# greysun/GraphEmbeddings

Measured on AMD Instinct MI355X. Metric: scored triples/sec/GPU (d=200), higher is better.
Workload: dtype f32

## Files before the change

### graphembeddings_amd/csrc/ge_common.h

```cpp
#pragma once
#include <hip/hip_runtime.h>
#include <hip/hip_ext.h>
#include <stdint.h>

#include <initializer_list>

#include "../../include/ge_hip.h"

namespace ge {

constexpr int kWave = 64;
constexpr int kBlock = 256;
constexpr int kMaxBlocks = 256 * 8;

template <int VEC> struct Vec;
template <> struct Vec<1> { using type = float; };
template <> struct Vec<2> { using type = float2; };
template <> struct Vec<4> { using type = float4; };

template <int VEC>
__device__ __forceinline__ void load_vec(const float* __restrict__ p, float (&r)[VEC]) {
  if constexpr (VEC == 4) {
    float4 v = *reinterpret_cast<const float4*>(p);
    r[0] = v.x; r[1] = v.y; r[2] = v.z; r[3] = v.w;
  } else if constexpr (VEC == 2) {
    float2 v = *reinterpret_cast<const float2*>(p);
    r[0] = v.x; r[1] = v.y;
  } else {
    r[0] = *p;
  }
}

template <int VEC>
__device__ __forceinline__ void store_vec(float* __restrict__ p, const float (&r)[VEC]) {
  if constexpr (VEC == 4) {
    *reinterpret_cast<float4*>(p) = make_float4(r[0], r[1], r[2], r[3]);
  } else if constexpr (VEC == 2) {
    *reinterpret_cast<float2*>(p) = make_float2(r[0], r[1]);
  } else {
    *p = r[0];
  }
}

template <int LPT>
__device__ __forceinline__ float group_sum(float v) {
#pragma unroll
  for (int m = LPT / 2; m >= 1; m >>= 1) v += __shfl_xor(v, m, kWave);
  return v;
}

__device__ __forceinline__ float clip_scale(float ss, float max_norm, float& inv) {
  inv = rsqrtf(ss);
  return fminf(inv, 1.0f / max_norm) * max_norm;
}

__device__ __forceinline__ float sigmoidf_dev(float x) { return 1.0f / (1.0f + expf(-x)); }

__device__ __forceinline__ void atomic_add_f32(float* p, float v) {
  __hip_atomic_fetch_add(p, v, __ATOMIC_RELAXED, __HIP_MEMORY_SCOPE_AGENT);
}

inline int grid_for(int64_t units, int units_per_block) {
  int64_t g = (units + units_per_block - 1) / units_per_block;
  if (g < 1) g = 1;
  if (g > kMaxBlocks) g = kMaxBlocks;
  return (int)g;
}

inline int launch_status() {
  hipError_t e = hipGetLastError();
  return e == hipSuccess ? 0 : (int)e;
}

inline size_t align_up(size_t v, size_t a) { return (v + a - 1) / a * a; }

inline unsigned sort_key_bits(int64_t n) {
  unsigned b = 1;
  while (b < 32 && ((uint64_t)1 << b) <= (uint64_t)n) ++b;
  return b;
}

inline bool aligned16(std::initializer_list<const void*> ptrs) {
  for (const void* p : ptrs) if ((uintptr_t)p & 15) return false;
  return true;
}

__device__ __forceinline__ uint32_t philox_w0(uint32_t c0, uint32_t c1, uint32_t c2, uint32_t c3,
                                              uint32_t k0, uint32_t k1) {
#pragma unroll
  for (int r = 0; r < 10; ++r) {
    uint64_t p0 = (uint64_t)0xD2511F53u * c0, p1 = (uint64_t)0xCD9E8D57u * c2;
    uint32_t n0 = (uint32_t)(p1 >> 32) ^ c1 ^ k0, n1 = (uint32_t)p1;
    uint32_t n2 = (uint32_t)(p0 >> 32) ^ c3 ^ k1, n3 = (uint32_t)p0;
    c0 = n0; c1 = n1; c2 = n2; c3 = n3;
// ... 50 lines not shown
```

### graphembeddings_amd/csrc/ge_complex.hip

```cpp
#include "ge_complex_dev.h"
#include "ge_launch.h"

namespace ge {

template <bool SPEC, int VEC, int LPT, int NITER>
__global__ __launch_bounds__(kBlock) void complex_score_kernel(
    const float* __restrict__ table, int64_t N, int d, const int32_t* __restrict__ triples, int64_t B,
    float max_norm, int apply_sigmoid, float* __restrict__ out, float label, float l2,
    const float* __restrict__ table_sumsq, int64_t ld) {
  constexpr int GPW = kWave / LPT;
  const int lane = threadIdx.x & (kWave - 1), sub = lane % LPT, grp = lane / LPT;
  const int64_t wave = ((int64_t)blockIdx.x * blockDim.x + threadIdx.x) >> 6;
  const int64_t nwaves = ((int64_t)gridDim.x * blockDim.x) >> 6;
  const int k = d >> 1, nvec = k / VEC;
  const float wscale = 1.0f / (float)d;
  for (int64_t base = wave * GPW; base < B; base += nwaves * GPW) {
    const int64_t g = base + grp;
    const bool live = g < B;
    int32_t hi = 0, ti = 0, ri = 0;
    if (live) { hi = triples[3 * g]; ti = triples[3 * g + 1]; ri = triples[3 * g + 2]; }
    const bool bad = bad3(N, hi, ti, ri);
    if (bad) { hi = ti = ri = 0; }
    Row<VEC, NITER> h, t, r;
    load_row_at<VEC, LPT, NITER>(table + (int64_t)hi * ld, k, nvec, sub, h);
// ... 118 lines not shown
          graw<SPEC, VEC, NITER>(X, xn[0], xn[1], xn[2], it, v, sub == 0, gre, gim);
          nre_[v] = kn.alpha * gre + kn.beta * xn[X].re[it][v];
          nim_[v] = kn.alpha * gim + kn.beta * xn[X].im[it][v];
        }
        if (same) {
#pragma unroll
          for (int v = 0; v < VEC; ++v) { pre_[v] += nre_[v]; pim_[v] += nim_[v]; }
        } else {
          if (dirN) {
#pragma unroll
            for (int v = 0; v < VEC; ++v) { nre_[v] += xn[X].re[it][v]; nim_[v] += xn[X].im[it][v]; }
          }
          store_vec<VEC>(gn + j * VEC, nre_);
          store_vec<VEC>(gn + k + j * VEC, nim_);
        }
        if (dirP) {
#pragma unroll
          for (int v = 0; v < VEC; ++v) { pre_[v] += xp[X].re[it][v]; pim_[v] += xp[X].im[it][v]; }
        }
        store_vec<VEC>(gp + j * VEC, pre_);
        store_vec<VEC>(gp + k + j * VEC, pim_);
      }
    }
  }
}


template <int CTRL>
__device__ __forceinline__ float dpp_add(float v) {
  return v + __int_as_float(__builtin_amdgcn_update_dpp(0, __float_as_int(v), CTRL, 0xF, 0xF, false));
}
template <int LPT>
__device__ __forceinline__ float group_sum_dpp(float v) {
  static_assert(LPT == 16 || LPT == 32 || LPT == 64, "lane group");
  v = dpp_add<0xB1>(v);
  v = dpp_add<0x4E>(v);
  v = dpp_add<0x141>(v);
  v = dpp_add<0x140>(v);
  if (LPT >= 32) v += __int_as_float(__builtin_amdgcn_ds_swizzle(__float_as_int(v), 0x401F));
  if (LPT >= 64) v += __shfl_xor(v, 32, kWave);
  return v;
}

template <int VEC, int LPT, int NITER>
__device__ __forceinline__ void load_row_clamped(const float* __restrict__ p, int k, int nvec, int sub, Row<VEC, NITER>& R) {
#pragma unroll
  for (int it = 0; it < NITER; ++it) {
    const int j = min(sub + it * LPT, nvec - 1);
    load_vec<VEC>(p + j * VEC, R.re[it]);
    load_vec<VEC>(p + k + j * VEC, R.im[it]);
  }
}

template <bool SPEC, bool SHARD, bool ORD, int VEC, int LPT, int NITER, bool PEER = false>
__global__ __launch_bounds__(kBlock, (VEC * NITER <= 4 ? 4 : 2)) void complex_hinge_grad_plan_kernel(
    const float* rows, int64_t N, int d, const int32_t* __restrict__ pos,
    const int32_t* __restrict__ neg, int64_t B, float margin, float lr, float max_norm,
    float* __restrict__ loss, int32_t* __restrict__ grad_idx, float* __restrict__ grad_val,
    const int32_t* __restrict__ slot_item, float* table_rw, ShardGrad sg, const int32_t* __restrict__ order) {
  constexpr int kSlotDirect = -2;
  constexpr int GPW = kWave / LPT;
  const int lane = threadIdx.x & (kWave - 1), sub = lane % LPT, grp = lane / LPT;
  const int wave = (int)(((int64_t)blockIdx.x * blockDim.x + threadIdx.x) >> 6);
  const int nwaves = (int)(((int64_t)gridDim.x * blockDim.x) >> 6);
  const int nB = (int)B;
  const int k = d >> 1, nvec = k / VEC;
  const float wscale = 1.0f / (float)d;
  const float neg_lr = -lr;
  float act[NITER];
#pragma unroll
  for (int it = 0; it < NITER; ++it) act[it] = (sub + it * LPT < nvec) ? 1.f : 0.f;
  const int per = ORD ? ((nB + nwaves - 1) / nwaves + GPW - 1) / GPW * GPW : 0;
  float racc_re[NITER][VEC], racc_im[NITER][VEC];
#pragma unroll
  for (int it = 0; it < NITER; ++it)
#pragma unroll
    for (int v = 0; v < VEC; ++v) { racc_re[it][v] = 0.f; racc_im[it][v] = 0.f; }
  int32_t cur_rel = -1;
  int cur_slot = -1;
  auto flush = [&]() {
    float* o = grad_val + (int64_t)cur_slot * d;
#pragma unroll
    for (int it = 0; it < NITER; ++it) {
      const int j = sub + it * LPT;
      if (j < nvec) {
        store_vec<VEC>(o + j * VEC, racc_re[it]);
        store_vec<VEC>(o + k + j * VEC, racc_im[it]);
      }
#pragma unroll
      for (int v = 0; v < VEC; ++v) { racc_re[it][v] = 0.f; racc_im[it][v] = 0.f; }
    }
    if (sub == 0) grad_idx[cur_slot] = cur_rel;
    cur_slot = -1;
  };
  typedef const __attribute__((address_space(4))) int32_t* kptr_t;
  auto kld = [](const int32_t* p, int i) -> int32_t { return ((kptr_t)(uintptr_t)p)[i]; };
  auto load_ids = [&](int g, int32_t (&raw)[5], int32_t (&tag)[5]) {
    if (SHARD) {
#pragma unroll
      for (int c = 0; c < 3; ++c) raw[c] = kld(sg.pos_src, 3 * g + c);
      raw[3] = kld(sg.neg_src, g); raw[4] = 0;
    } else {
#pragma unroll
      for (int c = 0; c < 3; ++c) raw[c] = kld(pos, 3 * g + c);
      raw[3] = kld(neg, 3 * g); raw[4] = kld(neg, 3 * g + 1);
    }
#pragma unroll
    for (int c = 0; c < 5; ++c) tag[c] = slot_item ? kld(slot_item, g * 6 + c) : 0;
  };
  auto pick = [&](const int32_t (&v)[GPW]) -> int32_t {
    int32_t r = v[0];
#pragma unroll
    for (int j = 1; j < GPW; ++j) r = (grp == j) ? v[j] : r;
    return r;
  };
  auto body = [&](const int g, const bool live, const int32_t (&raw)[5], const int32_t (&tag)[5], auto&& after_loads) {
    int32_t p0 = 0, p1 = 0, p2 = 0, c = 0;
    bool hs = false, bad;
    if (SHARD) {
      int32_t ns = -1;
      if (live) { p0 = raw[0]; p1 = raw[1]; p2 = raw[2]; ns = raw[3]; }
      bad = p0 < 0 || p1 < 0 || p2 < 0;
      hs = ns >= 0 && (ns & 1) == 0;
      c = ns >= 0 ? (ns >> 1) : p1;
    } else {
      int32_t n0 = 0, n1 = 0;
      if (live) { p0 = raw[0]; p1 = raw[1]; p2 = raw[2]; n0 = raw[3]; n1 = raw[4]; }
      bad = bad3(N, p0, p1, p2) || n0 < 0 || n1 < 0 || n0 >= N || n1 >= N;
      hs = n0 != p0;
      c = hs ? n0 : n1;
    }
    if (bad) { p0 = p1 = p2 = c = 0; hs = false; }
    const int32_t idF = hs ? p1 : p0, idV = hs ? p0 : p1;
    const float sigma = hs ? -1.f : 1.f;
    auto row_ptr = [&](int32_t id) -> const float* {
      if constexpr (SHARD && PEER) {
        if (id >= sg.R) {
          const int32_t o = id / sg.R - 1;
          return sg.peer[o & (kMaxPeers - 1)] + (int64_t)(id - sg.R * (o + 1)) * d;
        }
        return rows + (int64_t)id * d;
      } else if constexpr (SHARD) {
        const bool rem = id >= sg.R;
        const float* base = rem ? sg.staged : rows;
        return base + (int64_t)(rem ? id - sg.R : id) * d;
// ... 7 lines not shown
    load_row_clamped<VEC, LPT, NITER>(row_ptr(c), k, nvec, sub, xC);
    load_row_clamped<VEC, LPT, NITER>(row_ptr(p2), k, nvec, sub, xR);
    __builtin_amdgcn_sched_barrier(0);
    after_loads();
    __builtin_amdgcn_sched_barrier(0);
    const bool first_el = sub == 0;
    float wre[NITER][VEC], wim[NITER][VEC];
    float accP = 0.f, accN = 0.f, qF = 0.f, qV = 0.f, qC = 0.f, qR = 0.f;
#pragma unroll
    for (int it = 0; it < NITER; ++it) {
      float tP = 0.f, tN = 0.f;
#pragma unroll
      for (int v = 0; v < VEC; ++v) {
        const float a = xF.re[it][v], b = xF.im[it][v], cr = xR.re[it][v], di = xR.im[it][v];
        const float ds = sigma * di;
        float wr = a * cr - b * ds, wi = a * ds + b * cr;
        if (SPEC && it == 0 && v == 0 && first_el) { wr = a * cr; wi = b * di; }
        wre[it][v] = wr; wim[it][v] = wi;
        const float tp = wr * xV.re[it][v] + wi * xV.im[it][v], tn = wr * xC.re[it][v] + wi * xC.im[it][v];
        if (SPEC && !(it == 0 && v == 0 && first_el)) { tP += 2.f * tp; tN += 2.f * tn; }
        else { tP += tp; tN += tn; }
      }
      accP += act[it] * tP; accN += act[it] * tN;
    }
    {
      auto ssq = [&](const Row<VEC, NITER>& R) {
        float s = 0.f;
#pragma unroll
        for (int it = 0; it < NITER; ++it) {
          float t = 0.f;
#pragma unroll
          for (int v = 0; v < VEC; ++v) {
            const float q = R.re[it][v] * R.re[it][v] + R.im[it][v] * R.im[it][v];
            if (SPEC) t += (it == 0 && v == 0 && first_el) ? q : 2.f * q;
            else t += q;
          }
          s += act[it] * t;
        }
        return s;
      };
      qF = ssq(xF); qV = ssq(xV); qC = ssq(xC); qR = ssq(xR);
    }
    float ssF = group_sum_dpp<LPT>(qF), ssV = group_sum_dpp<LPT>(qV);
    float ssC = group_sum_dpp<LPT>(qC), ssR = group_sum_dpp<LPT>(qR);
    float srP = group_sum_dpp<LPT>(accP), srN = group_sum_dpp<LPT>(accN);
    if (SPEC) { ssF *= wscale; ssV *= wscale; ssC *= wscale; ssR *= wscale; srP *= wscale; srN *= wscale; }
    float invF, invV, invC, invR;
    const float scF = clip_scale(ssF, max_norm, invF), scV = clip_scale(ssV, max_norm, invV);
    const float scC = clip_scale(ssC, max_norm, invC), scR = clip_scale(ssR, max_norm, invR);
    const float sigP = sigmoidf_dev(srP * (hs ? scV : scF) * (hs ? scF : scV) * scR);
    const float sigN = sigmoidf_dev(srN * (hs ? scC : scF) * (hs ? scF : scC) * scR);
    const float pre = sigP - sigN + margin;
    const bool on = live && !bad && (pre >= 0.f);
    if (live && sub == 0) loss[g] = bad ? __builtin_nanf("") : fmaxf(pre, 0.f);
    const bool same = c == idV;
    const int slot0 = g * 6;
    const int32_t tagF = hs ? tag[1] : tag[0], tagV = hs ? tag[0] : tag[1], tagR = tag[2], tagC = hs ? tag[3] : tag[4];
    const bool dirF = slot_item && live && tagF == kSlotDirect, dirV = slot_item && live && tagV == kSlotDirect;
    const bool dirR = slot_item && live && tagR == kSlotDirect, dirC = slot_item && live && !same && tagC == kSlotDirect;
    const bool sndF = SHARD && slot_item && live && tagF <= -3, sndV = SHARD && slot_item && live && tagV <= -3;
    const bool sndR = SHARD && slot_item && live && tagR <= -3, sndC = SHARD && slot_item && live && !same && tagC <= -3;
    const bool accum = ORD && !dirR && !sndR;
    if (accum && live && cur_slot >= 0 && p2 != cur_rel) flush();
    if (live && sub == 0) {
      const int32_t giF = (on && !dirF && !sndF) ? idF : -1, giV = (on && !dirV && !sndV) ? idV : -1;
      const int32_t giC = (on && !same && !dirC && !sndC) ? c : -1;
      grad_idx[slot0] = hs ? giV : giF;
      grad_idx[slot0 + 1] = hs ? giF : giV;
      grad_idx[slot0 + 2] = (on && !dirR && !sndR && !accum) ? p2 : -1;
      grad_idx[slot0 + 3] = hs ? giC : -1;
      grad_idx[slot0 + 4] = hs ? -1 : giC;
      grad_idx[slot0 + 5] = -1;
    }
    if (!on) {
      if (SHARD && (sndF || sndV || sndR || sndC)) {
        float z[VEC];
#pragma unroll
        for (int v = 0; v < VEC; ++v) z[v] = 0.f;
        auto zero_row = [&](bool doit, int32_t tg) {
          if (!doit) return;
          float* o = sg.gsum + (int64_t)(-3 - tg) * d;
#pragma unroll
          for (int it = 0; it < NITER; ++it) {
            const int j = sub + it * LPT;
            if (j < nvec) { store_vec<VEC>(o + j * VEC, z); store_vec<VEC>(o + k + j * VEC, z); }
          }
        };
        zero_row(sndF, tagF); zero_row(sndV, tagV); zero_row(sndR, tagR); zero_row(sndC, tagC);
      }
      return;
    }
    const float cp = sigP * (1.f - sigP), cn = -sigN * (1.f - sigN);
    auto coef = [&](float cf, float P, float inv, float s_raw, float& alpha, float& beta) {
      const float A = cf * P;
      const bool active = inv <= 1.0f / max_norm;
      alpha = neg_lr * (active ? max_norm * A * inv : A);
      beta = active ? neg_lr * (-max_norm * A * s_raw * inv * inv * inv) : 0.f;
    };
    float aFp, bFp, aFn, bFn, aRp, bRp, aRn, bRn, aV, bV, aC, bC;
    coef(cp, scV * scR, invF, srP, aFp, bFp);
    coef(cn, scC * scR, invF, srN, aFn, bFn);
    coef(cp, scF * scV, invR, srP, aRp, bRp);
    coef(cn, scF * scC, invR, srN, aRn, bRn);
    coef(cp, scF * scR, invV, srP, aV, bV);
    coef(cn, scF * scR, invC, srN, aC, bC);
    const float bF = bFp + bFn, bR = bRp + bRn;
    if (same) { aV += aC; bV += bC; }
    const int hsi = hs ? 1 : 0;
    auto out_ptr = [&](bool dir, bool snd, int32_t tg, int32_t id, int slot) -> float* {
      return dir ? table_rw + (int64_t)id * d : (SHARD && snd) ? sg.gsum + (int64_t)(-3 - tg) * d : grad_val + (int64_t)slot * d;
    };
    {
      float* o = out_ptr(dirV, sndV, tagV, idV, slot0 + 1 - hsi);
#pragma unroll
      for (int it = 0; it < NITER; ++it) {
        const int j = sub + it * LPT;
        if (j >= nvec) continue;
        float ore[VEC], oim[VEC];
#pragma unroll
        for (int v = 0; v < VEC; ++v) {
          ore[v] = aV * wre[it][v] + bV * xV.re[it][v];
          oim[v] = aV * wim[it][v] + bV * xV.im[it][v];
          if (dirV) { ore[v] += xV.re[it][v]; oim[v] += xV.im[it][v]; }
        }
        store_vec<VEC>(o + j * VEC, ore);
        store_vec<VEC>(o + k + j * VEC, oim);
      }
    }
    if (!same) {
      float* o = out_ptr(dirC, sndC, tagC, c, slot0 + 4 - hsi);
#pragma unroll
      for (int it = 0; it < NITER; ++it) {
        const int j = sub + it * LPT;
        if (j >= nvec) continue;
        float ore[VEC], oim[VEC];
#pragma unroll
        for (int v = 0; v < VEC; ++v) {
          ore[v] = aC * wre[it][v] + bC * xC.re[it][v];
          oim[v] = aC * wim[it][v] + bC * xC.im[it][v];
          if (dirC) { ore[v] += xC.re[it][v]; oim[v] += xC.im[it][v]; }
        }
        store_vec<VEC>(o + j * VEC, ore);
        store_vec<VEC>(o + k + j * VEC, oim);
      }
    }
    {
      float* o = out_ptr(dirF, sndF, tagF, idF, slot0 + hsi);
#pragma unroll
      for (int it = 0; it < NITER; ++it) {
        const int j = sub + it * LPT;
        if (j >= nvec) continue;
        float ore[VEC], oim[VEC];
#pragma unroll
        for (int v = 0; v < VEC; ++v) {
          const float ur = aFp * xV.re[it][v] + aFn * xC.re[it][v], ui = aFp * xV.im[it][v] + aFn * xC.im[it][v];
          const float cr = xR.re[it][v], di = xR.im[it][v], ds = sigma * di;
          float gr = cr * ur + ds * ui, gim = cr * ui - ds * ur;
          if (SPEC && it == 0 && v == 0 && first_el) { gr = cr * ur; gim = di * ui; }
          ore[v] = gr + bF * xF.re[it][v];
          oim[v] = gim + bF * xF.im[it][v];
          if (dirF) { ore[v] += xF.re[it][v]; oim[v] += xF.im[it][v]; }
        }
        store_vec<VEC>(o + j * VEC, ore);
        store_vec<VEC>(o + k + j * VEC, oim);
      }
    }
    {
      float* o = out_ptr(dirR, sndR, tagR, p2, slot0 + 2);
#pragma unroll
      for (int it = 0; it < NITER; ++it) {
        const int j = sub + it * LPT;
        if (j >= nvec) continue;
        float ore[VEC], oim[VEC];
#pragma unroll
        for (int v = 0; v < VEC; ++v) {
          const float ur = aRp * xV.re[it][v] + aRn * xC.re[it][v], ui = aRp * xV.im[it][v] + aRn * xC.im[it][v];
          const float a = xF.re[it][v], b = xF.im[it][v];
          float gr = a * ur + b * ui, gim = sigma * (a * ui - b * ur);
          if (SPEC && it == 0 && v == 0 && first_el) { gr = a * ur; gim = b * ui; }
          ore[v] = gr + bR * xR.re[it][v];
          oim[v] = gim + bR * xR.im[it][v];
          if (dirR) { ore[v] += xR.re[it][v]; oim[v] += xR.im[it][v]; }
        }
        if (accum) {
#pragma unroll
          for (int v = 0; v < VEC; ++v) { racc_re[it][v] += ore[v]; racc_im[it][v] += oim[v]; }
        } else {
          store_vec<VEC>(o + j * VEC, ore);
          store_vec<VEC>(o + k + j * VEC, oim);
        }
      }
      if (accum) { cur_rel = p2; cur_slot = slot0 + 2; }
    }
  };
  const int wave_u = __builtin_amdgcn_readfirstlane(wave);
  const int start = ORD ? wave_u * per : wave_u * GPW, stop = ORD ? min(start + per, nB) : nB;
  const int stride = ORD ? GPW : nwaves * GPW;
  auto pair_at = [&](int i) -> int32_t {
    if (i >= stop) return 0;
    return ORD ? kld(order, i) : i;
  };
  int32_t gC[GPW], gN[GPW], rawS[GPW][5], tagS[GPW][5];
#pragma unroll
  for (int j = 0; j < GPW; ++j) { gC[j] = pair_at(start + j); gN[j] = pair_at(start + stride + j); }
#pragma unroll
  for (int j = 0; j < GPW; ++j) load_ids(gC[j], rawS[j], tagS[j]);
  for (int base = start; base < stop; base += stride) {
    const bool live = base + grp < stop;
    const int g = pick(gC);
    int32_t raw[5], tag[5];
#pragma unroll
    for (int c = 0; c < 5; ++c) {
      int32_t rv[GPW], tv[GPW];
#pragma unroll
      for (int j = 0; j < GPW; ++j) { rv[j] = rawS[j][c]; tv[j] = tagS[j][c]; }
      raw[c] = pick(rv); tag[c] = pick(tv);
    }
    body(g, live, raw, tag, [&]() {
#pragma unroll
      for (int j = 0; j < GPW; ++j) {
        gC[j] = gN[j];
        load_ids(gC[j], rawS[j], tagS[j]);
        gN[j] = pair_at(base + 2 * stride + j);
      }
    });
  }
  if constexpr (ORD) {
    constexpr int NG = (kBlock / kWave) * GPW, NF = NITER * VEC * LPT;
    __shared__ float part[NG][2 * NF];
    __shared__ int meta_rel[NG], meta_slot[NG];
    const int gi = (int)(threadIdx.x >> 6) * GPW + grp;
#pragma unroll
    for (int it = 0; it < NITER; ++it)
#pragma unroll
      for (int v = 0; v < VEC; ++v) {
        part[gi][(it * VEC + v) * LPT + sub] = racc_re[it][v];
        part[gi][NF + (it * VEC + v) * LPT + sub] = racc_im[it][v];
      }
    if (sub == 0) { meta_rel[gi] = cur_rel; meta_slot[gi] = cur_slot; }
    __syncthreads();
    if (cur_slot >= 0) {
      bool leader = true;
// ... 134 lines not shown
      case 1642: { CALL(1, 64, 2); } break;                                            \
      case 2161: { CALL(2, 16, 1); } break;                                            \
      case 2321: { CALL(2, 32, 1); } break;                                            \
      case 2641: { CALL(2, 64, 1); } break;                                            \
      case 2642: { CALL(2, 64, 2); } break;                                            \
      case 4161: { CALL(4, 16, 1); } break;                                            \
      case 4162: { CALL(4, 16, 2); } break;                                            \
      case 4322: { CALL(4, 32, 2); } break;                                            \
      case 4321: { CALL(4, 32, 1); } break;                                            \
      case 4641: { CALL(4, 64, 1); } break;                                            \
      case 4642: { CALL(4, 64, 2); } break;                                            \
      default: return GE_ENOTSUP;                                                      \
    }                                                                                  \
  } while (0)

#define GE_DISPATCH_SPEC(FLAG, S, CALL)                                                \
  do {                                                                                 \
    if (FLAG) { constexpr bool SP = true; GE_DISPATCH_SHAPE(S, 2, CALL); }             \
    else { constexpr bool SP = false; GE_DISPATCH_SHAPE(S, 2, CALL); }                 \
  } while (0)

int complex_score_launch(const float* table, int64_t N, int32_t d, const int32_t* triples, int64_t B,
                         float max_norm, int apply_sigmoid, float* out, hipStream_t st, int spectral, float label,
                         float l2, const float* table_sumsq, int64_t ld) {
  Shape s;
  if (ld <= 0) ld = d;
  if (!pick_shape(d, table, 2, s)) return (d <= 0 || (d & 1)) ? GE_EINVAL : GE_ENOTSUP;
  if (ld < d || (s.vec > 1 && ld % s.vec != 0)) return GE_EINVAL;
  if (B == 0) return 0;
  const int gpb = (kBlock / kWave) * (kWave / s.lpt);
  const int grid = grid_for(B, gpb);
#define CALL(V, L, NI) \
  hipLaunchKernelGGL((complex_score_kernel<SP, V, L, NI>), dim3(grid), dim3(kBlock), 0, st, table, N, d, triples, B, max_norm, apply_sigmoid, out, label, l2, table_sumsq, ld)
  GE_DISPATCH_SPEC(spectral, s, CALL);
#undef CALL
  return launch_status();
}

int complex_hinge_loss_launch(const float* table, int64_t N, int32_t d, const int32_t* pos,
                              const int32_t* neg, int64_t B, float margin, float max_norm, float* loss,
                              float* sig_out, hipStream_t st, int spectral) {
  Shape s;
  if (!pick_shape(d, table, 2, s)) return (d <= 0 || (d & 1)) ? GE_EINVAL : GE_ENOTSUP;
  if (B == 0) return 0;
  const int gpb = (kBlock / kWave) * (kWave / s.lpt);
  const int grid = grid_for(B, gpb);
#define CALL(V, L, NI) \
  hipLaunchKernelGGL((complex_hinge_loss_kernel<SP, V, L, NI>), dim3(grid), dim3(kBlock), 0, st, table, N, d, pos, neg, B, margin, max_norm, loss, sig_out)
  GE_DISPATCH_SPEC(spectral, s, CALL);
#undef CALL
  return launch_status();
}

int complex_hinge_grad_launch(const float* rows, int64_t N, int32_t d, const int32_t* pos,
                              const int32_t* neg, int64_t B, float margin, float lr, float max_norm,
                              float* loss, int32_t* grad_idx, float* grad_val, hipStream_t st,
                              hipEvent_t ev_start, hipEvent_t ev_stop, const int32_t* slot_item, float* table_rw,
                              int spectral, const int32_t* order) {
  Shape s;
  if (!pick_shape(d, rows, 2, s)) return (d <= 0 || (d & 1)) ? GE_EINVAL : GE_ENOTSUP;
  while (s.vec > 1 && (reinterpret_cast<uintptr_t>(grad_val) % (s.vec * 4)) != 0) return GE_EINVAL;
  if ((slot_item != nullptr) != (table_rw != nullptr)) return GE_EINVAL;
  if (B == 0) return 0;
  const int gpb = (kBlock / kWave) * (kWave / s.lpt);
  const int grid = grid_for(B, gpb);
#define CALL(V, L, NI) \
  hipExtLaunchKernelGGL((complex_hinge_grad_kernel<SP, V, L, NI>), dim3(grid), dim3(kBlock), 0, st, ev_start, ev_stop, 0, rows, N, d, pos, neg, B, margin, lr, max_norm, loss, grad_idx, grad_val, slot_item, table_rw)
#define CALLO(V, L, NI) \
  hipExtLaunchKernelGGL((complex_hinge_grad_plan_kernel<SP, false, true, V, L, NI>), dim3(grid), dim3(kBlock), 0, st, ev_start, ev_stop, 0, rows, N, d, pos, neg, B, margin, lr, max_norm, loss, grad_idx, grad_val, slot_item, table_rw, ShardGrad{}, order)
#define CALLP(V, L, NI) \
  hipExtLaunchKernelGGL((complex_hinge_grad_plan_kernel<SP, false, false, V, L, NI>), dim3(grid), dim3(kBlock), 0, st, ev_start, ev_stop, 0, rows, N, d, pos, neg, B, margin, lr, max_norm, loss, grad_idx, grad_val, slot_item, table_rw, ShardGrad{}, nullptr)
  if (order) { GE_DISPATCH_SPEC(spectral, s, CALLO); }
  else if (slot_item) { GE_DISPATCH_SPEC(spectral, s, CALLP); }
  else { GE_DISPATCH_SPEC(spectral, s, CALL); }
#undef CALLP
#undef CALLO
#undef CALL
  return launch_status();
}

int shard_hinge_grad_launch(float* shard, int32_t d, const float* staged, const int32_t* pos_src, const int32_t* neg_src,
                            const int32_t* slot_item, int32_t R, int64_t B, float margin, float lr, float max_norm,
                            float* loss, int32_t* grad_idx, float* grad_val, float* gsum, int spectral, hipStream_t st,
                            hipEvent_t ev_start, hipEvent_t ev_stop, const int32_t* order, const float* const* peers, int n_peers) {
  Shape s;
  if (!pick_shape(d, shard, 2, s)) return (d <= 0 || (d & 1)) ? GE_EINVAL : GE_ENOTSUP;
  for (const void* q : {(const void*)grad_val, (const void*)staged, (const void*)gsum})
    if (q && (reinterpret_cast<uintptr_t>(q) % (s.vec * 4)) != 0) return GE_EINVAL;
  if (B == 0) return 0;
  const int gpb = (kBlock / kWave) * (kWave / s.lpt);
  const int grid = grid_for(B, gpb);
  ShardGrad sg{staged, R, pos_src, neg_src, gsum, {}};
  if (peers) {
    if (staged || n_peers > kMaxPeers) return GE_EINVAL;
    for (int i = 0; i < kMaxPeers; ++i) sg.peer[i] = i < n_peers ? peers[i] : nullptr;
  }
#define CALL(V, L, NI) \
  hipExtLaunchKernelGGL((complex_hinge_grad_plan_kernel<SP, true, ORDF, V, L, NI, PEERF>), dim3(grid), dim3(kBlock), 0, st, ev_start, ev_stop, 0, shard, (int64_t)R, d, nullptr, nullptr, B, margin, lr, max_norm, loss, grad_idx, grad_val, slot_item, shard, sg, order)
  if (peers) {
    constexpr bool PEERF = true;
    if (order) { constexpr bool ORDF = true; GE_DISPATCH_SPEC(spectral, s, CALL); }
    else { constexpr bool ORDF = false; GE_DISPATCH_SPEC(spectral, s, CALL); }
  } else {
    constexpr bool PEERF = false;
    if (order) { constexpr bool ORDF = true; GE_DISPATCH_SPEC(spectral, s, CALL); }
    else { constexpr bool ORDF = false; GE_DISPATCH_SPEC(spectral, s, CALL); }
  }
#undef CALL
  return launch_status();
}

int complex_logloss_grad_launch(const float* rows, int64_t N, int32_t d, const int32_t* triples,
                                const float* labels, int64_t M, float lr, float max_norm, float l2,
                                const float* table_sumsq, float* loss, int32_t* grad_idx, float* grad_val,
                                hipStream_t st, const int32_t* negs, int64_t B, float row_scale, float neg_lr_eff,
                                hipEvent_t ev_start, hipEvent_t ev_stop) {
  Shape s;
  if (!pick_shape(d, rows, 2, s)) return (d <= 0 || (d & 1)) ? GE_EINVAL : GE_ENOTSUP;
  if ((reinterpret_cast<uintptr_t>(grad_val) % (s.vec * 4)) != 0) return GE_EINVAL;
  if (M == 0) return 0;
  if (!negs) neg_lr_eff = -lr;
  const int gpb = (kBlock / kWave) * (kWave / s.lpt);
  const int grid = grid_for(M, gpb);
#define CALL(V, L, NI) \
// ... 22 lines not shown
```

### graphembeddings_amd/csrc/ge_train.hip

```cpp
#include "ge_prep.h"
#include "ge_launch.h"
#include <cmath>

namespace ge {

__global__ __launch_bounds__(kPrepThreads) void train_prepare_kernel(
    const int32_t* __restrict__ triples, int64_t T, int64_t first_row, int64_t B, int64_t s0,
    const int32_t* __restrict__ id_to_type, int64_t N, const int64_t* __restrict__ type_offsets,
    int32_t n_types, const int32_t* __restrict__ type_ids, uint64_t seed, uint64_t global_step0,
    int32_t padded_size, int32_t mode, int direct, int n_pass, int bits, int negs, int32_t* __restrict__ prep) {
  extern __shared__ __attribute__((aligned(16))) unsigned long long keys[];
  const PrepLayout L = prep_layout(B, negs);
  const int P = (int)L.P, R = P / kPrepThreads;
  unsigned* hist = reinterpret_cast<unsigned*>(keys + P);
  int* wtot = reinterpret_cast<int*>(hist + kPrepWaves * kMaxRadix);
  const int tid = threadIdx.x, lane = tid & (kWave - 1), wave = tid >> 6;
  const int sub = blockIdx.y;
  const int64_t s = s0 + blockIdx.x;
  const int32_t* pos = triples + 3 * step_row(first_row, T, B, s);
  int32_t* rec = prep + (int64_t)blockIdx.x * L.stride;
  int32_t* neg = rec;
  int32_t* slot_item = rec + L.off_slot;
  int32_t* subrec = rec + L.off_sub + sub * L.sub_stride;
  int32_t* items = subrec + L.off_items;
// ... 81 lines not shown
  int rs_loc[16];
  {
    int carry = -1;
#pragma unroll
    for (int r = 0; r < 16; ++r) {
      if (r < R) {
        const int i = wave * seg + r * kWave + lane;
        const unsigned long long kk = keys[i], kp = key_at(i - 1);
        const bool head = kk != kInvalid && (i == 0 || (uint32_t)(kp >> 32) != (uint32_t)(kk >> 32));
        const int m = max(wave_incl_max(head ? i : -1, lane), carry);
        rs_loc[r] = m;
        carry = __shfl(m, kWave - 1, kWave);
      }
    }
    if (lane == 0) wtot[wave] = carry;
  }
  __syncthreads();
  int prev_max = -1;
  for (int w = 0; w < wave; ++w) prev_max = max(prev_max, wtot[w]);
  __syncthreads();
  unsigned start_mask = 0;
  int idx_loc[16];
  {
    int carry = 0;
#pragma unroll
    for (int r = 0; r < 16; ++r) {
      if (r < R) {
        const int i = wave * seg + r * kWave + lane;
        const unsigned long long kk = keys[i], kp = key_at(i - 1), kn = key_at(i + 1);
        const bool valid = kk != kInvalid;
        const uint32_t row = (uint32_t)(kk >> 32);
        const bool head = valid && (i == 0 || (uint32_t)(kp >> 32) != row);
        const bool sole = direct && head && !(kn != kInvalid && (uint32_t)(kn >> 32) == row);
        const int rs = max(rs_loc[r], prev_max);
        rs_loc[r] = rs;
        const bool start = valid && ((i - rs) % kItemCap) == 0 && !sole;
        if (start) start_mask |= 1u << r;
        if (sole) slot_item[(uint32_t)kk] = kSlotDirect;
        const int incl = wave_incl_add(start ? 1 : 0, lane) + carry;
        idx_loc[r] = incl - (start ? 1 : 0);
        carry = __shfl(incl, kWave - 1, kWave);
      }
    }
    if (lane == 0) wtot[wave] = carry;
  }
  __syncthreads();
  int prev_items = 0, total = 0;
  for (int w = 0; w < kPrepWaves; ++w) { if (w < wave) prev_items += wtot[w]; total += wtot[w]; }
  if (tid == 0) subrec[0] = total;
#pragma unroll
  for (int r = 0; r < 16; ++r) {
    if (r < R && ((start_mask >> r) & 1u)) {
      const int i = wave * seg + r * kWave + lane;
      const uint32_t row = (uint32_t)(keys[i] >> 32);
      const int idx = prev_items + idx_loc[r];
      int e = i + 1;
      while (e < P && (e - i) < kItemCap && keys[e] != kInvalid && (uint32_t)(keys[e] >> 32) == row) ++e;
      const bool more = (e < P && keys[e] != kInvalid && (uint32_t)(keys[e] >> 32) == row);
      const bool multi = (i != rs_loc[r]) || more;
      items[2 * idx] = (int32_t)row;
      items[2 * idx + 1] = (e - i) | (multi ? (1 << 30) : 0);
#pragma unroll
      for (int j = 0; j < kItemCap; ++j)
        islots[idx * kItemCap + j] = (i + j < e) ? (int32_t)(uint32_t)keys[i + j] : -1;
    }
  }
}

template <int NJ, bool COND, bool DET = false>
__global__ __launch_bounds__(kBlock) void apply_sorted_kernel(
    float* __restrict__ table, int d, const int32_t* __restrict__ sub0, int64_t sub_stride, int off_items,
    int off_islots, const int32_t* __restrict__ grad_idx, const float* grad_val, int split,
    float* __restrict__ out2) {
  const int lane = threadIdx.x & (kWave - 1);
  const int wave = (int)(((int64_t)blockIdx.x * blockDim.x + threadIdx.x) >> 6);
  const int nwaves = (int)(((int64_t)gridDim.x * blockDim.x) >> 6);
  const int32_t* subrec = sub0 + (int64_t)blockIdx.y * sub_stride;
  const int32_t* items = subrec + off_items;
  const int32_t* islots = subrec + off_islots;
  const int n_items = subrec[0];
  for (int w = wave; w < n_items; w += nwaves) {
    const int row = items[2 * w], cm = items[2 * w + 1];
    int slot_v = (lane < kItemCap) ? islots[w * kItemCap + lane] : -1;
    const int cnt = cm & 0x3FFFFFFF;
    const bool multi = (cm >> 30) & 1;
    const bool away = row >= split;
    float* dst = away ? out2 + (int64_t)(row - split) * d : table + (int64_t)row * d;
    float base[NJ];
#pragma unroll
    for (int j = 0; j < NJ; ++j) {
      const int c = lane + kWave * j;
      base[j] = (!multi && !away && c < d) ? dst[c] : 0.f;
    }
    const bool act_v = slot_v >= 0 && (!grad_idx || grad_idx[slot_v] >= 0);
    if (slot_v < 0) slot_v = 0;
    const unsigned long long live = __ballot(act_v);
    const bool park = DET && multi && !away;
    if (live == 0ull && !(away && !multi) && !park) continue;
    float acc[NJ];
#pragma unroll
    for (int j = 0; j < NJ; ++j) acc[j] = 0.f;
    for (int o = 0; o < cnt; o += 4) {
      int sl[4];
      bool on[4];
#pragma unroll
      for (int q = 0; q < 4; ++q) {
        const int src_lane = (o + q < cnt) ? (o + q) : o;
        sl[q] = __shfl(slot_v, src_lane, kWave);
        on[q] = (o + q < cnt) && ((live >> (o + q)) & 1ull);
      }
      float v[4][NJ];
#pragma unroll
      for (int q = 0; q < 4; ++q) {
        const float* src = grad_val + (int64_t)sl[q] * d;
#pragma unroll
        for (int j = 0; j < NJ; ++j) {
          const int c = lane + kWave * j;
// ... 82 lines not shown
  for (int h = wv; h < nh; h += kWv) {
    const int k0 = heads[h];
    const int row = (subrec + off_items)[2 * k0];
    int fs = 0;
    const bool mine = item_at(k0, lane, row, fs);
    const int n = __popcll(__ballot(mine));
    if (n == kWave) continue;
    float acc[NJ];
#pragma unroll
    for (int j = 0; j < NJ; ++j) acc[j] = 0.f;
    add_rows(fs, n, acc);
    float* dst = table + (int64_t)row * d;
#pragma unroll
    for (int j = 0; j < NJ; ++j) { const int c = lane + kWave * j; if (c < d) dst[c] = dst[c] + acc[j]; }
    if (lane == 0) heads[h] = -1;
  }
  __syncthreads();
  for (int h = 0; h < nh; ++h) {
    const int k0 = heads[h];
    if (k0 < 0) continue;
    const int row = (subrec + off_items)[2 * k0];
    float acc[NJ];
#pragma unroll
    for (int j = 0; j < NJ; ++j) acc[j] = 0.f;
    for (int r0 = wv; ; r0 += kWv * kWave) {
      int fs = 0;
      const bool mine = item_at(k0, r0 + kWv * lane, row, fs);
      const int n = __popcll(__ballot(mine));
      add_rows(fs, n, acc);
      if (n < kWave) break;
    }
    if (wv > 0) {
#pragma unroll
      for (int j = 0; j < NJ; ++j) part[wv - 1][j * kWave + lane] = acc[j];
    }
    __syncthreads();
    if (wv == 0) {
      float* dst = table + (int64_t)row * d;
#pragma unroll
      for (int j = 0; j < NJ; ++j) {
        const int c = lane + kWave * j;
        float tot = acc[j];
#pragma unroll
        for (int w2 = 0; w2 < kWv - 1; ++w2) tot += part[w2][j * kWave + lane];
        if (c < d) dst[c] = dst[c] + tot;
      }
    }
    __syncthreads();
  }
  __syncthreads();
  }
}

template <int VW, int NJ, bool DET = false>
__global__ __launch_bounds__(kBlock) void apply_rows_kernel(
    float* __restrict__ table, int d, const int32_t* __restrict__ sub0, int64_t sub_stride, int off_items,
    int off_islots, const int32_t* __restrict__ grad_idx, const float* grad_val, int split,
    float* __restrict__ out2) {
  typedef const __attribute__((address_space(4))) int32_t* kptr_t;
  constexpr int RG0 = 16 / (VW * NJ);
  constexpr int RG = RG0 > kItemCap ? kItemCap : (RG0 < 2 ? 2 : RG0);
  const int lane = threadIdx.x & (kWave - 1);
  const int wave = __builtin_amdgcn_readfirstlane((int)(((int64_t)blockIdx.x * blockDim.x + threadIdx.x) >> 6));
  const int nwaves = (int)(((int64_t)gridDim.x * blockDim.x) >> 6);
  const int32_t* subrec = sub0 + (int64_t)blockIdx.y * sub_stride;
  const kptr_t items = (kptr_t)(uintptr_t)(subrec + off_items);
  const int32_t* islots = subrec + off_islots;
  const int n_items = ((kptr_t)(uintptr_t)subrec)[0];
  int col[NJ];
  bool ok[NJ];
#pragma unroll
  for (int j = 0; j < NJ; ++j) { col[j] = VW * (lane + kWave * j); ok[j] = col[j] < d; if (!ok[j]) col[j] = 0; }
  for (int w = wave; w < n_items; w += nwaves) {
    const int row = items[2 * w], cm = items[2 * w + 1];
    int slot_v = (lane < kItemCap) ? islots[w * kItemCap + lane] : -1;
    const int cnt = cm & 0x3FFFFFFF;
    const bool multi = (cm >> 30) & 1;
    const bool away = row >= split;
    float* dst = away ? out2 + (int64_t)(row - split) * d : table + (int64_t)row * d;
    if (multi) {
      constexpr int ND = VW * NJ;
      const bool act_v = slot_v >= 0 && (!grad_idx || grad_idx[slot_v] >= 0);
      const unsigned long long lv = __ballot(act_v);
      const bool park = DET && !away;
      if (lv == 0ull && !park) continue;
      float a[ND];
#pragma unroll
      for (int j = 0; j < ND; ++j) a[j] = 0.f;
      for (int o = 0; o < cnt; o += 4) {
        float v[4][ND];
#pragma unroll
        for (int q = 0; q < 4; ++q)
          if (o + q < cnt && ((lv >> (o + q)) & 1ull)) {
            const float* src = grad_val + (int64_t)__builtin_amdgcn_readlane(slot_v, o + q) * d;
#pragma unroll
            for (int j = 0; j < ND; ++j) { const int c = lane + kWave * j; v[q][j] = src[c < d ? c : 0]; }
          }
#pragma unroll
        for (int q = 0; q < 4; ++q)
          if (o + q < cnt && ((lv >> (o + q)) & 1ull)) {
#pragma unroll
            for (int j = 0; j < ND; ++j) a[j] += v[q][j];
          }
      }
      float* parked = const_cast<float*>(grad_val) + (int64_t)__builtin_amdgcn_readlane(slot_v, 0) * d;
#pragma unroll
      for (int j = 0; j < ND; ++j) {
        const int c = lane + kWave * j;
        if (c < d) { if (park) parked[c] = a[j]; else atomic_add_f32(dst + c, a[j]); }
      }
      continue;
    }
    float base[NJ][VW];
#pragma unroll
    for (int j = 0; j < NJ; ++j) {
      if (!away) load_vec<VW>(dst + col[j], base[j]);
      else {
#pragma unroll
        for (int e = 0; e < VW; ++e) base[j][e] = 0.f;
      }
    }
    float acc[NJ][VW];
#pragma unroll
    for (int j = 0; j < NJ; ++j)
#pragma unroll
      for (int e = 0; e < VW; ++e) acc[j][e] = 0.f;
    unsigned long long live = 0ull;
    bool have_live = false;
    for (int o = 0; o < cnt; o += RG) {
      float v[RG][NJ][VW];
      if (!have_live) {
        const bool act_v = slot_v >= 0 && (!grad_idx || grad_idx[slot_v] >= 0);
        live = __ballot(act_v);
        have_live = true;
      }
#pragma unroll
      for (int q = 0; q < RG; ++q)
        if (o + q < cnt && ((live >> (o + q)) & 1ull)) {
          const int sl = __builtin_amdgcn_readlane(slot_v, o + q);
          const float* src = grad_val + (int64_t)sl * d;
#pragma unroll
          for (int j = 0; j < NJ; ++j) load_vec<VW>(src + col[j], v[q][j]);
        }
#pragma unroll
      for (int q = 0; q < RG; ++q)
        if (o + q < cnt && ((live >> (o + q)) & 1ull)) {
#pragma unroll
          for (int j = 0; j < NJ; ++j)
#pragma unroll
            for (int e = 0; e < VW; ++e) acc[j][e] += v[q][j][e];
        }
    }
    if (live == 0ull && !away) continue;
#pragma unroll
    for (int j = 0; j < NJ; ++j) {
      if (!ok[j]) continue;
      float o_[VW];
#pragma unroll
      for (int e = 0; e < VW; ++e) o_[e] = base[j][e] + acc[j][e];
      store_vec<VW>(dst + col[j], o_);
    }
  }
}

int apply_items_launch(float* table, int d, const TileGeom& G, const int32_t* step_rec, const int32_t* gidx,
                       const float* gval, int split, float* out2, hipStream_t st, hipEvent_t ev_start, hipEvent_t ev_stop,
                       int det) {
  const int grid = grid_for(G.P, kBlock / kWave);
  const int nj = (d + kWave - 1) / kWave;
  const dim3 g((unsigned)grid, (unsigned)G.n_sub);
  auto hot = [&]() -> int {
    const dim3 gh((unsigned)((G.P + kWave - 1) / kWave), (unsigned)G.n_sub);
#define LH(NJ) hipLaunchKernelGGL((hot_rows_kernel<NJ>), gh, dim3(kHotBlock), 0, st, table, d, step_rec + G.off_sub, G.sub_stride, G.off_items, G.off_islots, G.n_sub, gval)
    if (nj <= 1) LH(1); else if (nj <= 2) LH(2); else if (nj <= 4) LH(4); else if (nj <= 8) LH(8); else LH(16);
#undef LH
    return launch_status();
  };
  if (det && nj > 16) return GE_ENOTSUP;
#define LA(NJ)                                                                                                             \
  {                                                                                                                        \
    if (G.n_sub > 1) hipExtLaunchKernelGGL((apply_sorted_kernel<NJ, true>), g, dim3(kBlock), 0, st, ev_start, ev_stop, 0, table, d, step_rec + G.off_sub, G.sub_stride, G.off_items, G.off_islots, gidx, gval, split, out2); \
    else if (det) { hipExtLaunchKernelGGL((apply_sorted_kernel<NJ, false, true>), g, dim3(kBlock), 0, st, ev_start, ev_stop, 0, table, d, step_rec + G.off_sub, G.sub_stride, G.off_items, G.off_islots, gidx, gval, split, out2); return hot(); } \
    else hipExtLaunchKernelGGL((apply_sorted_kernel<NJ, false>), g, dim3(kBlock), 0, st, ev_start, ev_stop, 0, table, d, step_rec + G.off_sub, G.sub_stride, G.off_items, G.off_islots, gidx, gval, split, out2); \
  }
  if (gidx != nullptr || G.n_sub > 1) {
    auto al = [](const void* q, int a) { return q == nullptr || reinterpret_cast<uintptr_t>(q) % a == 0; };
    const int vw = (d % 4 == 0 && al(table, 16) && al(gval, 16) && al(out2, 16)) ? 4 : (d % 2 == 0 && al(table, 8) && al(gval, 8) && al(out2, 8)) ? 2 : 1;
    const int njr = (d / vw + kWave - 1) / kWave;
    const dim3 g((unsigned)(G.n_sub > 1 ? grid_for((G.P + 7) / 8, kBlock / kWave) : grid), (unsigned)G.n_sub);
#define LR(VW, NJ)                                                                                                       \
    {                                                                                                                    \
      if (det) {                                                                                                         \
        hipExtLaunchKernelGGL((apply_rows_kernel<VW, NJ, true>), g, dim3(kBlock), 0, st, ev_start, ev_stop, 0, table, d, \
                              step_rec + G.off_sub, G.sub_stride, G.off_items, G.off_islots, gidx, gval, split, out2);   \
        return hot();                                                                                                    \
      }                                                                                                                  \
      hipExtLaunchKernelGGL((apply_rows_kernel<VW, NJ>), g, dim3(kBlock), 0, st, ev_start, ev_stop, 0, table, d, \
                            step_rec + G.off_sub, G.sub_stride, G.off_items, G.off_islots, gidx, gval, split, out2);     \
      return launch_status();                                                                                            \
    }
    if (vw == 4) { if (njr <= 1) LR(4, 1) else if (njr <= 2) LR(4, 2) else if (njr <= 4) LR(4, 4) }
    else if (vw == 2) { if (njr <= 1) LR(2, 1) else if (njr <= 2) LR(2, 2) else if (njr <= 4) LR(2, 4) else if (njr <= 8) LR(2, 8) }
    else { if (njr <= 1) LR(1, 1) else if (njr <= 2) LR(1, 2) else if (njr <= 4) LR(1, 4) else if (njr <= 8) LR(1, 8) else if (njr <= 16) LR(1, 16) }
#undef LR
  }
  if (nj <= 1) LA(1) else if (nj <= 2) LA(2) else if (nj <= 4) LA(4) else if (nj <= 8) LA(8) else if (nj <= 16) LA(16)
  else return GE_ENOTSUP;
#undef LA
  return launch_status();
}

static int apply_sorted_launch(float* table, int d, const PrepLayout& L, const int32_t* step_rec, const int32_t* gidx,
                               const float* gval, hipStream_t st, hipEvent_t ev_start, hipEvent_t ev_stop, int det = 0) {
  return apply_items_launch(table, d, geom_of(L), step_rec, gidx, gval, 0x7FFFFFFF, nullptr, st, ev_start, ev_stop, det);
}

size_t hinge_ws_bytes(int64_t B, int32_t d) {
  return align_up(sizeof(int32_t) * 6 * (size_t)B, 256) + align_up(sizeof(float) * 6 * (size_t)B * (size_t)d, 256);
}

static bool train_fast_ok(int64_t B, int32_t d) { return B >= 1 && B <= (int64_t)1 << 24 && d <= 1024; }

static int64_t prep_chunk_steps(int64_t B, int64_t negs = 0) {
  const int64_t u = negs > 0 ? (1 + negs) * B : B;
  int64_t c = (32 * kSub) / (u < kSub ? kSub : u);
  const int64_t floor_steps = u <= 32768 ? 16 : u <= 4 * 65536 ? 8 : 2;
  return c < floor_steps ? floor_steps : c;
}

static size_t grad_region_bytes(int64_t B, int32_t d) {
  return align_up(sizeof(float) * 6 * (size_t)B * (size_t)d, 256);
}
static int grad_ring(int64_t B, int32_t d) {
  const size_t reg = grad_region_bytes(B, d);
  size_t r = ((size_t)64 << 20) / reg + 1;
  if (r < 2) r = 2;
  if (r > 16) r = 16;
  if (r < 4 && 4 * reg <= ((size_t)160 << 20)) r = 4;
  return (int)r;
}
static size_t train_grad_bytes(int64_t B, int32_t d) {
  return align_up(sizeof(int32_t) * 6 * (size_t)B, 256) + (size_t)grad_ring(B, d) * grad_region_bytes(B, d);
}
static size_t prep_chunk_bytes(int64_t B, int64_t negs = 0) {
  return align_up(sizeof(int32_t) * (size_t)prep_chunk_steps(B, negs) * (size_t)prep_layout(B, negs).stride, 256);
}
size_t train_ws_bytes(int64_t B, int32_t d) {
  if (!train_fast_ok(B, d)) return hinge_ws_bytes(B, d);
  return train_grad_bytes(B, d) + 2 * prep_chunk_bytes(B) + prep_big_scratch_bytes(B, 0, prep_chunk_steps(B));
}

// ... 350 lines not shown
```

Before: 543.7 million.

## Use write-through sc1 stores for gradient and apply outputs, vectorize item build

Adds store helpers that emit global stores with the sc1 cache-policy bit (or relaxed agent-scope atomics for scalars). It turns them on by default for the hinge-gradient plan kernel's gradient, index and loss outputs, and for the apply-rows kernel when there is one sub-tile and no second output. The aim is to change how these producer writes interact with the cache hierarchy so the consumer kernel reads them with less overhead. Separately, the item-build loop now reads a fixed window of keys into registers with no data-dependent while loop, and writes items and slots with vector int2/int4 stores. The inline asm carries an s_nop and depends on the hardware's cache semantics. The fixed-window read may touch keys past the run, so key_at must handle bounds.

```diff
diff --git a/graphembeddings_amd/csrc/ge_common.h b/graphembeddings_amd/csrc/ge_common.h
--- a/graphembeddings_amd/csrc/ge_common.h
+++ b/graphembeddings_amd/csrc/ge_common.h
@@ -40,6 +40,31 @@
   } else {
     *p = r[0];
   }
+}
+
+template <int VEC>
+__device__ __forceinline__ void store_vec_wt(float* p, const float (&r)[VEC]) {
+  if constexpr (VEC == 4) {
+    typedef float f4 __attribute__((ext_vector_type(4)));
+    const f4 v = {r[0], r[1], r[2], r[3]};
+    asm volatile("global_store_dwordx4 %0, %1, off sc1\n\ts_nop 1" : : "v"(p), "v"(v) : "memory");
+  } else if constexpr (VEC == 2) {
+    typedef float f2 __attribute__((ext_vector_type(2)));
+    const f2 v = {r[0], r[1]};
+    asm volatile("global_store_dwordx2 %0, %1, off sc1" : : "v"(p), "v"(v) : "memory");
+  } else {
+    __hip_atomic_store(p, r[0], __ATOMIC_RELAXED, __HIP_MEMORY_SCOPE_AGENT);
+  }
+}
+template <bool WT, int VEC>
+__device__ __forceinline__ void store_vec_as(float* p, const float (&r)[VEC]) {
+  if constexpr (WT) store_vec_wt<VEC>(p, r);
+  else store_vec<VEC>(p, r);
+}
+template <bool WT, typename T>
+__device__ __forceinline__ void store_as(T* p, T v) {
+  if constexpr (WT) __hip_atomic_store(p, v, __ATOMIC_RELAXED, __HIP_MEMORY_SCOPE_AGENT);
+  else *p = v;
 }
 
 template <int LPT>
diff --git a/graphembeddings_amd/csrc/ge_complex.hip b/graphembeddings_amd/csrc/ge_complex.hip
--- a/graphembeddings_amd/csrc/ge_complex.hip
+++ b/graphembeddings_amd/csrc/ge_complex.hip
@@ -194,7 +194,7 @@
   }
 }
 
-template <bool SPEC, bool SHARD, bool ORD, int VEC, int LPT, int NITER, bool PEER = false>
+template <bool SPEC, bool SHARD, bool ORD, int VEC, int LPT, int NITER, bool PEER = false, bool WT = false>
 __global__ __launch_bounds__(kBlock, (VEC * NITER <= 4 ? 4 : 2)) void complex_hinge_grad_plan_kernel(
     const float* rows, int64_t N, int d, const int32_t* __restrict__ pos,
     const int32_t* __restrict__ neg, int64_t B, float margin, float lr, float max_norm,
@@ -226,13 +226,13 @@
     for (int it = 0; it < NITER; ++it) {
       const int j = sub + it * LPT;
       if (j < nvec) {
-        store_vec<VEC>(o + j * VEC, racc_re[it]);
-        store_vec<VEC>(o + k + j * VEC, racc_im[it]);
+        store_vec_as<WT, VEC>(o + j * VEC, racc_re[it]);
+        store_vec_as<WT, VEC>(o + k + j * VEC, racc_im[it]);
       }
 #pragma unroll
       for (int v = 0; v < VEC; ++v) { racc_re[it][v] = 0.f; racc_im[it][v] = 0.f; }
     }
-    if (sub == 0) grad_idx[cur_slot] = cur_rel;
+    if (sub == 0) store_as<WT>(grad_idx + cur_slot, cur_rel);
     cur_slot = -1;
   };
   typedef const __attribute__((address_space(4))) int32_t* kptr_t;
@@ -346,7 +346,7 @@
     const float sigN = sigmoidf_dev(srN * (hs ? scC : scF) * (hs ? scF : scC) * scR);
     const float pre = sigP - sigN + margin;
     const bool on = live && !bad && (pre >= 0.f);
-    if (live && sub == 0) loss[g] = bad ? __builtin_nanf("") : fmaxf(pre, 0.f);
+    if (live && sub == 0) store_as<WT>(loss + g, bad ? __builtin_nanf("") : fmaxf(pre, 0.f));
     const bool same = c == idV;
     const int slot0 = g * 6;
     const int32_t tagF = hs ? tag[1] : tag[0], tagV = hs ? tag[0] : tag[1], tagR = tag[2], tagC = hs ? tag[3] : tag[4];
@@ -359,12 +359,12 @@
     if (live && sub == 0) {
       const int32_t giF = (on && !dirF && !sndF) ? idF : -1, giV = (on && !dirV && !sndV) ? idV : -1;
       const int32_t giC = (on && !same && !dirC && !sndC) ? c : -1;
-      grad_idx[slot0] = hs ? giV : giF;
-      grad_idx[slot0 + 1] = hs ? giF : giV;
-      grad_idx[slot0 + 2] = (on && !dirR && !sndR && !accum) ? p2 : -1;
-      grad_idx[slot0 + 3] = hs ? giC : -1;
-      grad_idx[slot0 + 4] = hs ? -1 : giC;
-      grad_idx[slot0 + 5] = -1;
+      store_as<WT>(grad_idx + slot0, hs ? giV : giF);
+      store_as<WT>(grad_idx + slot0 + 1, hs ? giF : giV);
+      store_as<WT>(grad_idx + slot0 + 2, (on && !dirR && !sndR && !accum) ? p2 : -1);
+      store_as<WT>(grad_idx + slot0 + 3, hs ? giC : -1);
+      store_as<WT>(grad_idx + slot0 + 4, hs ? -1 : giC);
+      store_as<WT>(grad_idx + slot0 + 5, -1);
     }
     if (!on) {
       if (SHARD && (sndF || sndV || sndR || sndC)) {
@@ -417,8 +417,8 @@
           oim[v] = aV * wim[it][v] + bV * xV.im[it][v];
           if (dirV) { ore[v] += xV.re[it][v]; oim[v] += xV.im[it][v]; }
         }
-        store_vec<VEC>(o + j * VEC, ore);
-        store_vec<VEC>(o + k + j * VEC, oim);
+        store_vec_as<WT, VEC>(o + j * VEC, ore);
+        store_vec_as<WT, VEC>(o + k + j * VEC, oim);
       }
     }
     if (!same) {
@@ -434,8 +434,8 @@
           oim[v] = aC * wim[it][v] + bC * xC.im[it][v];
           if (dirC) { ore[v] += xC.re[it][v]; oim[v] += xC.im[it][v]; }
         }
-        store_vec<VEC>(o + j * VEC, ore);
-        store_vec<VEC>(o + k + j * VEC, oim);
+        store_vec_as<WT, VEC>(o + j * VEC, ore);
+        store_vec_as<WT, VEC>(o + k + j * VEC, oim);
       }
     }
     {
@@ -455,8 +455,8 @@
           oim[v] = gim + bF * xF.im[it][v];
           if (dirF) { ore[v] += xF.re[it][v]; oim[v] += xF.im[it][v]; }
         }
-        store_vec<VEC>(o + j * VEC, ore);
-        store_vec<VEC>(o + k + j * VEC, oim);
+        store_vec_as<WT, VEC>(o + j * VEC, ore);
+        store_vec_as<WT, VEC>(o + k + j * VEC, oim);
       }
     }
     {
@@ -480,8 +480,8 @@
 #pragma unroll
           for (int v = 0; v < VEC; ++v) { racc_re[it][v] += ore[v]; racc_im[it][v] += oim[v]; }
         } else {
-          store_vec<VEC>(o + j * VEC, ore);
-          store_vec<VEC>(o + k + j * VEC, oim);
+          store_vec_as<WT, VEC>(o + j * VEC, ore);
+          store_vec_as<WT, VEC>(o + k + j * VEC, oim);
         }
       }
       if (accum) { cur_rel = p2; cur_slot = slot0 + 2; }
@@ -722,6 +722,9 @@
   return launch_status();
 }
 
+#ifndef GE_WT_GRAD
+#define GE_WT_GRAD true
+#endif
 int complex_hinge_grad_launch(const float* rows, int64_t N, int32_t d, const int32_t* pos,
                               const int32_t* neg, int64_t B, float margin, float lr, float max_norm,
                               float* loss, int32_t* grad_idx, float* grad_val, hipStream_t st,
@@ -739,7 +742,7 @@
 #define CALLO(V, L, NI) \
   hipExtLaunchKernelGGL((complex_hinge_grad_plan_kernel<SP, false, true, V, L, NI>), dim3(grid), dim3(kBlock), 0, st, ev_start, ev_stop, 0, rows, N, d, pos, neg, B, margin, lr, max_norm, loss, grad_idx, grad_val, slot_item, table_rw, ShardGrad{}, order)
 #define CALLP(V, L, NI) \
-  hipExtLaunchKernelGGL((complex_hinge_grad_plan_kernel<SP, false, false, V, L, NI>), dim3(grid), dim3(kBlock), 0, st, ev_start, ev_stop, 0, rows, N, d, pos, neg, B, margin, lr, max_norm, loss, grad_idx, grad_val, slot_item, table_rw, ShardGrad{}, nullptr)
+  hipExtLaunchKernelGGL((complex_hinge_grad_plan_kernel<SP, false, false, V, L, NI, false, GE_WT_GRAD>), dim3(grid), dim3(kBlock), 0, st, ev_start, ev_stop, 0, rows, N, d, pos, neg, B, margin, lr, max_norm, loss, grad_idx, grad_val, slot_item, table_rw, ShardGrad{}, nullptr)
   if (order) { GE_DISPATCH_SPEC(spectral, s, CALLO); }
   else if (slot_item) { GE_DISPATCH_SPEC(spectral, s, CALLP); }
   else { GE_DISPATCH_SPEC(spectral, s, CALL); }
diff --git a/graphembeddings_amd/csrc/ge_train.hip b/graphembeddings_amd/csrc/ge_train.hip
--- a/graphembeddings_amd/csrc/ge_train.hip
+++ b/graphembeddings_amd/csrc/ge_train.hip
@@ -157,17 +157,23 @@
   for (int r = 0; r < 16; ++r) {
     if (r < R && ((start_mask >> r) & 1u)) {
       const int i = wave * seg + r * kWave + lane;
-      const uint32_t row = (uint32_t)(keys[i] >> 32);
       const int idx = prev_items + idx_loc[r];
-      int e = i + 1;
-      while (e < P && (e - i) < kItemCap && keys[e] != kInvalid && (uint32_t)(keys[e] >> 32) == row) ++e;
-      const bool more = (e < P && keys[e] != kInvalid && (uint32_t)(keys[e] >> 32) == row);
+      unsigned long long kv[kItemCap + 1];
+#pragma unroll
+      for (int j = 0; j <= kItemCap; ++j) kv[j] = key_at(i + j);
+      const uint32_t row = (uint32_t)(kv[0] >> 32);
+      int cnt = 0;
+#pragma unroll
+      for (int j = 0; j < kItemCap; ++j) cnt += (uint32_t)(kv[j] >> 32) == row ? 1 : 0;
+      const bool more = (uint32_t)(kv[kItemCap] >> 32) == row;
       const bool multi = (i != rs_loc[r]) || more;
-      items[2 * idx] = (int32_t)row;
-      items[2 * idx + 1] = (e - i) | (multi ? (1 << 30) : 0);
-#pragma unroll
-      for (int j = 0; j < kItemCap; ++j)
-        islots[idx * kItemCap + j] = (i + j < e) ? (int32_t)(uint32_t)keys[i + j] : -1;
+      *reinterpret_cast<int2*>(items + 2 * idx) = make_int2((int32_t)row, cnt | (multi ? (1 << 30) : 0));
+      int sl[kItemCap];
+#pragma unroll
+      for (int j = 0; j < kItemCap; ++j) sl[j] = j < cnt ? (int32_t)(uint32_t)kv[j] : -1;
+      int4* o = reinterpret_cast<int4*>(islots + idx * kItemCap);
+#pragma unroll
+      for (int q = 0; q < kItemCap / 4; ++q) o[q] = make_int4(sl[4 * q], sl[4 * q + 1], sl[4 * q + 2], sl[4 * q + 3]);
     }
   }
 }
@@ -356,7 +362,7 @@
   }
 }
 
-template <int VW, int NJ, bool DET = false>
+template <int VW, int NJ, bool DET = false, bool WT = false>
 __global__ __launch_bounds__(kBlock) void apply_rows_kernel(
     float* __restrict__ table, int d, const int32_t* __restrict__ sub0, int64_t sub_stride, int off_items,
     int off_islots, const int32_t* __restrict__ grad_idx, const float* grad_val, int split,
@@ -462,11 +468,14 @@
       float o_[VW];
 #pragma unroll
       for (int e = 0; e < VW; ++e) o_[e] = base[j][e] + acc[j][e];
-      store_vec<VW>(dst + col[j], o_);
-    }
-  }
-}
-
+      store_vec_as<WT, VW>(dst + col[j], o_);
+    }
+  }
+}
+
+#ifndef GE_WT_APPLY
+#define GE_WT_APPLY true
+#endif
 int apply_items_launch(float* table, int d, const TileGeom& G, const int32_t* step_rec, const int32_t* gidx,
                        const float* gval, int split, float* out2, hipStream_t st, hipEvent_t ev_start, hipEvent_t ev_stop,
                        int det) {
@@ -492,6 +501,7 @@
     const int vw = (d % 4 == 0 && al(table, 16) && al(gval, 16) && al(out2, 16)) ? 4 : (d % 2 == 0 && al(table, 8) && al(gval, 8) && al(out2, 8)) ? 2 : 1;
     const int njr = (d / vw + kWave - 1) / kWave;
     const dim3 g((unsigned)(G.n_sub > 1 ? grid_for((G.P + 7) / 8, kBlock / kWave) : grid), (unsigned)G.n_sub);
+    const bool wt = GE_WT_APPLY && G.n_sub == 1 && out2 == nullptr;
 #define LR(VW, NJ)                                                                                                       \
     {                                                                                                                    \
       if (det) {                                                                                                         \
@@ -499,8 +509,12 @@
                               step_rec + G.off_sub, G.sub_stride, G.off_items, G.off_islots, gidx, gval, split, out2);   \
         return hot();                                                                                                    \
       }                                                                                                                  \
-      hipExtLaunchKernelGGL((apply_rows_kernel<VW, NJ>), g, dim3(kBlock), 0, st, ev_start, ev_stop, 0, table, d, \
-                            step_rec + G.off_sub, G.sub_stride, G.off_items, G.off_islots, gidx, gval, split, out2);     \
+      if (wt)                                                                                                            \
+        hipExtLaunchKernelGGL((apply_rows_kernel<VW, NJ, false, true>), g, dim3(kBlock), 0, st, ev_start, ev_stop, 0,   \
+                              table, d, step_rec + G.off_sub, G.sub_stride, G.off_items, G.off_islots, gidx, gval, split, out2); \
+      else                                                                                                               \
+        hipExtLaunchKernelGGL((apply_rows_kernel<VW, NJ>), g, dim3(kBlock), 0, st, ev_start, ev_stop, 0, table, d,     \
+                              step_rec + G.off_sub, G.sub_stride, G.off_items, G.off_islots, gidx, gval, split, out2);   \
       return launch_status();                                                                                            \
     }
     if (vw == 4) { if (njr <= 1) LR(4, 1) else if (njr <= 2) LR(4, 2) else if (njr <= 4) LR(4, 4) }
```

New measurement: 550.0 million, median of 6. 1.01x the previous value.
